# yuchencong/quantum_circuits_symmetry_breaking_based_on_tneq-qc

Hardware: NVIDIA B200
Metric: samples/sec for QCTN fwd+bwd contraction (higher is better)
Workload: dtype f32

## Files before the change

quantum_circuits_symmetry_breaking_based_on_tneq-qc_b200/csrc/tnq_ladder.cu:

```cuda
#include <cuda_runtime.h>
#include <stdint.h>
#include <stdlib.h>

#include <string>

#include "tneq_b200.h"
#include "tnq_ladder_core.cuh"

extern int tnq_internal_fail(const std::string& msg);
extern int tnq_internal_cuda_fail(cudaError_t e, const char* what);
extern void tnq_internal_count_launch();

namespace {

using namespace tnq_ladder;

constexpr int WARPS_FWD = 16;
constexpr int WARPS_TRAIN = 8;

template <int K>
__host__ __device__ constexpr int cst_floats(int n) {
    return ((n - 1) * Dims<K>::CSTEP + Dims<K>::K2 + 3) / 4 * 4;
}

template <int K, int MODE>
__global__ void __maxnreg__(MODE == 0 ? 128 : 255)
tnq_ladder_kernel(const __grid_constant__ Args a, long long B, long long ngroups, const float* __restrict__ seed,
                  float* __restrict__ values, float* __restrict__ gparts, float* __restrict__ lparts,
                  float* __restrict__ ckpt, float log_scale, float inv_count) {
    using D = Dims<K>;
    extern __shared__ __align__(16) float sm[];
    const int n = a.n;
    const int ncst = (n - 1) * D::CSTEP + D::K2;
    for (int i = threadIdx.x; i < ncst; i += blockDim.x) sm[i] = const_pool_element<K>(a, i);
    constexpr int WSZ = MODE == 0 ? D::WARP_FWD : D::WARP_TRAIN;
    const int warp = threadIdx.x >> 5, lane = threadIdx.x & 31, wpc = blockDim.x >> 5;
    float* wb = sm + cst_floats<K>(n) + warp * WSZ;
    for (int i = lane; i < WSZ; i += 32) wb[i] = 0.f;
    __syncthreads();
    const long long wg = (long long)warp * gridDim.x + blockIdx.x;
    const long long wtotal = (long long)wpc * gridDim.x;
    if (wg >= ngroups) return;
    WarpCtx<K> c;
    c.cst = sm;
    c.E = wb;
    c.U = c.E + D::E_SZ;
    c.T2 = c.U + D::U_SZ;
    c.M = c.T2 + D::T2_SZ;
    c.V = c.M + D::M_SZ;
    c.D = c.V + D::V_SZ;
    c.dT2 = c.D + D::E_SZ;
    c.args = &a;
    c.B = B;
    c.seed = seed;
    c.values = values;
    c.log_scale = log_scale;
    c.inv_count = inv_count;
    c.ckE = nullptr, c.ckT2 = nullptr, c.gpart = nullptr;
    if (MODE != 0) {
        const int ng = D::grad_floats(n);
        c.gpart = gparts + (size_t)wg * ng;
        for (int i = lane; i < ng; i += 32) c.gpart[i] = 0.f;
        c.ckE = ckpt + (size_t)wg * D::ckpt_floats(n);
        c.ckT2 = c.ckE + (size_t)(n - 2) * D::E_SZ;
        __syncwarp();
    }
    LaneState<K> st;
    st.loss = 0.f;
    st.mnext = 0.f;
    for (long long g = wg; g < ngroups; g += wtotal) ladder_group<K, MODE>(c, st, lane, g * D::SPW);
    if (MODE == 1) lparts[wg * 32 + lane] = st.loss;
}

template <int K>
__global__ void __launch_bounds__(256)
// ... 27 lines not shown
    __syncthreads();
    if (w != 0 || e >= ng) return;
    float s = 0.f;
#pragma unroll
    for (int i = 0; i < 8; ++i) s += part[i][lane];
    const int nX = (n - 1) * D::K4, nB = (n - 1) * D::K3;
    if (e < nX) {
        a.gradX[e / D::K4][e % D::K4] = s;
    } else if (e < nX + nB) {
        const int q = (e - nX) / D::K3, r = (e - nX) % D::K3;
        if (q == 0) return;
        const int cc = r / D::K2, ee = (r / K) % K, f = r % K;
        for (int d = 0; d < K; ++d) a.gradA[q][((cc * K + d) * K + ee) * K + f] = s * __ldg(a.state[q + 1] + d);
    } else if (e < nX + nB + D::K2) {
        const int ef = e - nX - nB;
        for (int cc = 0; cc < K; ++cc)
            for (int d = 0; d < K; ++d)
                a.gradA[0][(cc * K + d) * D::K2 + ef] = s * __ldg(a.state[0] + cc) * __ldg(a.state[1] + d);
    }
}

struct Geometry {
    int grid, wpc;
    long long ngroups, nwarps;
    size_t smem;
};

template <int K>
Geometry geometry(int n, long long B, int mode, int sms) {
    using D = Dims<K>;
    Geometry g;
    g.ngroups = (B + D::SPW - 1) / D::SPW;
    int wmax = mode == 0 ? WARPS_FWD : WARPS_TRAIN;
    {
        int dev = 0, smem_max = 227 * 1024;
        if (cudaGetDevice(&dev) == cudaSuccess) cudaDeviceGetAttribute(&smem_max, cudaDevAttrMaxSharedMemoryPerBlockOptin, dev);
        const long long per_warp = (long long)sizeof(float) * (mode == 0 ? D::WARP_FWD : D::WARP_TRAIN);
        const long long fit = ((long long)smem_max - (long long)sizeof(float) * cst_floats<K>(n)) / per_warp;
        if (fit < wmax) wmax = fit < 1 ? 1 : (int)fit;
    }
    long long wpc = (g.ngroups + sms - 1) / sms;
    g.wpc = (int)(wpc < 1 ? 1 : (wpc > wmax ? wmax : wpc));
    long long grid = (g.ngroups + g.wpc - 1) / g.wpc;
    g.grid = (int)(grid > sms ? sms : grid);
    g.nwarps = (long long)g.grid * g.wpc;
    if (g.nwarps > g.ngroups) g.nwarps = g.ngroups;
    g.smem = sizeof(float) * ((size_t)cst_floats<K>(n) + (size_t)g.wpc * (mode == 0 ? D::WARP_FWD : D::WARP_TRAIN));
    return g;
}

template <int K>
size_t workspace_bytes(int n, long long B, int mode, int sms) {
    using D = Dims<K>;
    if (mode == 0) return 256;
    const Geometry g = geometry<K>(n, B, mode, sms);
    const size_t nw = (size_t)g.grid * g.wpc;
    return sizeof(float) * nw * ((size_t)D::grad_floats(n) + 32 + (size_t)D::ckpt_floats(n)) + 256;
}

template <int K, int MODE>
int launch_mode(const Args& a, const Geometry& g, long long B, const float* seed, float* values, float* gparts,
                float* lparts, float* ckpt, float log_scale, cudaStream_t st) {
    cudaError_t e = cudaFuncSetAttribute(tnq_ladder_kernel<K, MODE>, cudaFuncAttributeMaxDynamicSharedMemorySize, (int)g.smem);
    if (e != cudaSuccess) return tnq_internal_cuda_fail(e, "cudaFuncSetAttribute(ladder)");
    tnq_ladder_kernel<K, MODE><<<g.grid, g.wpc * 32, g.smem, st>>>(a, B, g.ngroups, seed, values, gparts, lparts, ckpt,
                                                                    log_scale, 1.0f / (float)B);
    tnq_internal_count_launch();
    return 0;
}

template <int K>
int launch_ladder(const Args& a, long long B, int mode, const float* seed, float* values, float* loss, float log_scale,
                  void* workspace, long long ws_bytes, cudaStream_t st) {
    using D = Dims<K>;
    int dev = 0, sms = 148;
    cudaGetDevice(&dev);
    cudaDeviceGetAttribute(&sms, cudaDevAttrMultiProcessorCount, dev);
    const Geometry g = geometry<K>(a.n, B, mode, sms);
    float *gparts = nullptr, *lparts = nullptr, *ckpt = nullptr;
    if (mode != 0) {
        if ((size_t)ws_bytes < workspace_bytes<K>(a.n, B, mode, sms)) return tnq_internal_fail("tnq_mps_ladder: workspace too small");
        const size_t nw = (size_t)g.grid * g.wpc;
        gparts = reinterpret_cast<float*>(workspace);
        lparts = gparts + nw * D::grad_floats(a.n);
        ckpt = lparts + nw * 32;
    }
    int rc;
    if (mode == 0)
        rc = launch_mode<K, 0>(a, g, B, seed, values, gparts, lparts, ckpt, log_scale, st);
    else if (mode == 1)
        rc = launch_mode<K, 1>(a, g, B, seed, values, gparts, lparts, ckpt, log_scale, st);
    else
        rc = launch_mode<K, 2>(a, g, B, seed, values, gparts, lparts, ckpt, log_scale, st);
    if (rc) return rc;
    if (mode != 0) {
        const int nblk = (D::grad_floats(a.n) + 31) / 32;
        tnq_ladder_finalize_kernel<K><<<nblk + (mode == 1 ? 1 : 0), 256, 0, st>>>(a, gparts, lparts, (int)g.nwarps,
                                                                                  mode == 1 ? loss : nullptr);
        tnq_internal_count_launch();
    }
    const cudaError_t e = cudaGetLastError();
    if (e != cudaSuccess) return tnq_internal_cuda_fail(e, "tnq_mps_ladder launch");
    return 0;
}

}

extern "C" {

static bool use_second_generation(int K) {
    const char* v = getenv("TNQ_LADDER_V2");
    return K == 3 && v != nullptr && v[0] == '1';
}

int64_t tnq_mps_ladder_workspace_bytes(int K, int n, int64_t B, int mode) {
    if (use_second_generation(K)) return tnq_mps_ladder2_workspace_bytes(n, B, mode);
    int dev = 0, sms = 148;
    if (cudaGetDevice(&dev) == cudaSuccess) cudaDeviceGetAttribute(&sms, cudaDevAttrMultiProcessorCount, dev);
    if (n < 3 || n > MAXQ || B <= 0) return 256;
    return (int64_t)(K == 2 ? workspace_bytes<2>(n, B, mode, sms) : workspace_bytes<3>(n, B, mode, sms));
}

int tnq_mps_ladder(int K, int n, const float* const* cores_a, const float* const* cores_x, const float* const* states,
                   const float* const* mx, const int64_t* mx_stride, int64_t B, int mode, const float* seed,
                   float* values, float* loss, float* const* grads_a, float* const* grads_x, double log_scale,
                   void* workspace, int64_t workspace_bytes, void* stream) {
    if (use_second_generation(K))
        return tnq_mps_ladder2(n, cores_a, cores_x, states, mx, mx_stride, B, mode, seed, values, loss, grads_a, grads_x,
                               log_scale, workspace, workspace_bytes, stream);
    if (n < 3 || n > MAXQ) return tnq_internal_fail("tnq_mps_ladder: between 3 and " + std::to_string(MAXQ) + " qubits");
    if (K != 2 && K != 3) return tnq_internal_fail("tnq_mps_ladder: edge rank must be 2 or 3");
    if (!cores_a || !cores_x || !states || !mx || !mx_stride || B <= 0 || mode < 0 || mode > 2)
        return tnq_internal_fail("tnq_mps_ladder: bad arguments");
    if (mode != 0 && (!grads_a || !grads_x || !workspace)) return tnq_internal_fail("tnq_mps_ladder: gradients need grads[] and a workspace");
    if (mode == 0 && !values) return tnq_internal_fail("tnq_mps_ladder: mode 0 needs values");
    if (mode == 1 && !loss) return tnq_internal_fail("tnq_mps_ladder: mode 1 needs loss");
    if (mode == 2 && !seed) return tnq_internal_fail("tnq_mps_ladder: mode 2 needs a seed");
    Args a;
    a.n = n;
    for (int q = 0; q < MAXQ; ++q) {
        const bool hq = q < n, hc = q < n - 1;
        a.state[q] = hq ? states[q] : nullptr;
        a.mx[q] = hq ? mx[q] : nullptr;
        a.mx_stride[q] = hq ? mx_stride[q] : 0;
        a.coreA[q] = hc ? cores_a[q] : nullptr;
        a.coreX[q] = hc ? cores_x[q] : nullptr;
        a.gradA[q] = (hc && mode != 0) ? grads_a[q] : nullptr;
        a.gradX[q] = (hc && mode != 0) ? grads_x[q] : nullptr;
        if (hq && (!states[q] || !mx[q])) return tnq_internal_fail("tnq_mps_ladder: null pointer at qubit " + std::to_string(q));
        if (hc && (!cores_a[q] || !cores_x[q] || (mode != 0 && (!grads_a[q] || !grads_x[q]))))
            return tnq_internal_fail("tnq_mps_ladder: null core pointer at qubit " + std::to_string(q));
    }
    cudaStream_t st = (cudaStream_t)stream;
    if (K == 2) return launch_ladder<2>(a, B, mode, seed, values, loss, (float)log_scale, workspace, workspace_bytes, st);
    return launch_ladder<3>(a, B, mode, seed, values, loss, (float)log_scale, workspace, workspace_bytes, st);
}

}
```

quantum_circuits_symmetry_breaking_based_on_tneq-qc_b200/csrc/tnq_ladder_core.cuh:

```cuda
#pragma once

#include <math.h>
#include <stdint.h>

#ifdef __CUDACC__
#define TNQ_HOSTDEV __host__ __device__
#define TNQ_HD __device__ __forceinline__
#define TNQ_UNROLL _Pragma("unroll")
#define TNQ_NOUNROLL _Pragma("unroll 1")
#define TNQ_UNROLL3 _Pragma("unroll 3")
#else
#define TNQ_HOSTDEV
#define TNQ_HD inline
#define TNQ_UNROLL
#define TNQ_NOUNROLL
#define TNQ_UNROLL3
#endif

#include "tnq_f2.cuh"

namespace tnq_ladder {

constexpr int MAXQ = 64;

template <int K>
struct Dims {
    static constexpr int K2 = K * K, K3 = K2 * K, K4 = K2 * K2;
    static constexpr int IPS = K2;
    static constexpr int SPW = 32 / IPS;
    static constexpr int LANES = SPW * IPS;
    static constexpr int PITCH = K == 3 ? 85 : 16;
    static constexpr int SST = K == 3 ? 765 : 67;
    static constexpr int UP = 4;
    static constexpr int UQ = (K2 + 3) / 4 * 4;
    static constexpr int USZ = K3 * UP > K2 * UQ ? K3 * UP : K2 * UQ;
    static constexpr int XTP = (K2 + 3) / 4 * 4;
    static constexpr int BSP = 4;
    static constexpr int LP = LANES | 1;
    static constexpr int BTP = (K2 + 3) / 4 * 4;
    static constexpr int OFF_XN = 0, OFF_XT = (K4 + 3) / 4 * 4, OFF_BS = OFF_XT + K2 * XTP;
    static constexpr int OFF_BT = (OFF_BS + K2 * BSP + 3) / 4 * 4;
    static constexpr int CSTEP = (OFF_BT + K * BTP + 3) / 4 * 4;
    static constexpr int E_SZ = (SPW * SST + 3) / 4 * 4;
    static constexpr int U_SZ = SPW * USZ;
    static constexpr int T2_SZ = (SPW * K4 + 3) / 4 * 4;
    static constexpr int M_SZ = (SPW * K2 + 3) / 4 * 4;
    static constexpr int V_SZ = 64;
    static constexpr int WARP_FWD = E_SZ + U_SZ + T2_SZ + M_SZ + V_SZ;
    static constexpr int WARP_TRAIN = WARP_FWD + E_SZ + T2_SZ;
    static_assert(SPW * SST >= K4 * LP, "environment buffer doubles as the lane-reduction scratch");
    static_assert(USZ >= K4, "U buffer doubles as the X-gradient side buffer");
    TNQ_HOSTDEV static constexpr int ckpt_floats(int n) { return (n - 2) * (E_SZ + T2_SZ); }
    TNQ_HOSTDEV static constexpr int grad_floats(int n) { return ((n - 1) * K4 + (n - 1) * K3 + K2 + 3) / 4 * 4; }
};

struct Args {
    const float* coreA[MAXQ];
    const float* coreX[MAXQ];
    const float* state[MAXQ];
    const float* mx[MAXQ];
    long long mx_stride[MAXQ];
    float* gradA[MAXQ];
    float* gradX[MAXQ];
    int n;
};

template <int N>
struct Vec {
    static constexpr int NP = N / 2;
    F2 p[NP > 0 ? NP : 1];
    float s;
    TNQ_HD float get(int i) const { return i < 2 * NP ? ((i & 1) ? p[i >> 1].hi : p[i >> 1].lo) : s; }
    TNQ_HD void set(int i, float v) {
        if (i < 2 * NP) {
            if (i & 1) p[i >> 1].hi = v; else p[i >> 1].lo = v;
        } else {
            s = v;
        }
    }
    TNQ_HD void zero() {
        TNQ_UNROLL
        for (int i = 0; i < NP; ++i) p[i] = F2{0.f, 0.f};
        s = 0.f;
    }
};
template <int N>
TNQ_HD void axpy(Vec<N>& acc, float s, const Vec<N>& x) {
    TNQ_UNROLL
    for (int i = 0; i < Vec<N>::NP; ++i) acc.p[i] = fma2(x.p[i], s, acc.p[i]);
    if (N & 1) acc.s = fmaf(x.s, s, acc.s);
}
template <int N>
TNQ_HD float dot(const Vec<N>& a, const Vec<N>& b, float init) {
    F2 t{init, 0.f};
    TNQ_UNROLL
    for (int i = 0; i < Vec<N>::NP; ++i) t = fma2(a.p[i], b.p[i], t);
    if (N & 1) t.lo = fmaf(a.s, b.s, t.lo);
    return t.lo + t.hi;
}
template <int N>
TNQ_HD void vload(Vec<N>& v, const float* p) {
    float t[(N + 3) / 4 * 4];
#ifdef __CUDA_ARCH__
    TNQ_UNROLL
    for (int i = 0; i < (N + 3) / 4; ++i) {
        const float4 q = *reinterpret_cast<const float4*>(p + 4 * i);
        t[4 * i] = q.x, t[4 * i + 1] = q.y, t[4 * i + 2] = q.z, t[4 * i + 3] = q.w;
    }
#else
    for (int i = 0; i < (N + 3) / 4 * 4; ++i) t[i] = p[i];
#endif
    TNQ_UNROLL
    for (int i = 0; i < N; ++i) v.set(i, t[i]);
}

template <int K>
struct LaneState {
// ... 36 lines not shown
        }
    } else {
        TNQ_UNROLL
        for (int i = 0; i < N; ++i) o[i] = p[i];
    }
#else
    for (int i = 0; i < N; ++i) o[i] = p[i];
#endif
}
template <int N>
TNQ_HD void stv(float* p, const float (&o)[N]) {
#ifdef __CUDA_ARCH__
    if constexpr (N % 4 == 0) {
        TNQ_UNROLL
        for (int i = 0; i < N; i += 4) *reinterpret_cast<float4*>(p + i) = make_float4(o[i], o[i + 1], o[i + 2], o[i + 3]);
    } else if constexpr (N % 2 == 0) {
        TNQ_UNROLL
        for (int i = 0; i < N; i += 2) *reinterpret_cast<float2*>(p + i) = make_float2(o[i], o[i + 1]);
    } else {
        TNQ_UNROLL
        for (int i = 0; i < N; ++i) p[i] = o[i];
    }
#else
    for (int i = 0; i < N; ++i) p[i] = o[i];
#endif
}

TNQ_HD float ldg_f(const float* p) {
#ifdef __CUDA_ARCH__
    return __ldg(p);
#else
    return *p;
#endif
}

template <int K>
TNQ_HD float load_m(const WarpCtx<K>& c, int q, long long b, int it) {
    return b < c.B ? ldg_f(c.args->mx[q] + b * c.args->mx_stride[q] + it) : 0.f;
}

template <int K>
TNQ_HD void gather_epg(const float* e, Vec<Dims<K>::K2> (&Epg)[K][K]) {
    using D = Dims<K>;
    TNQ_UNROLL
    for (int cc = 0; cc < K; ++cc)
        TNQ_UNROLL
        for (int ee = 0; ee < K; ++ee)
            TNQ_UNROLL
            for (int l = 0; l < K; ++l)
                TNQ_UNROLL
                for (int n = 0; n < K; ++n) Epg[cc][ee].set(l * K + n, e[(cc * K + l) * D::PITCH + n * D::K3 + ee * K]);
}
template <int K>
TNQ_HD void contract_t1(const float* Bs, const Vec<Dims<K>::K2> (&Epg)[K][K], Vec<Dims<K>::K2> (&T1)[K]) {
    using D = Dims<K>;
    TNQ_UNROLL
    for (int f = 0; f < K; ++f) T1[f].zero();
    TNQ_UNROLL
    for (int cc = 0; cc < K; ++cc)
        TNQ_UNROLL
        for (int ee = 0; ee < K; ++ee) {
            float bs[D::BSP];
            ldv<D::BSP>(Bs + (cc * K + ee) * D::BSP, bs);
            TNQ_UNROLL
            for (int f = 0; f < K; ++f) axpy(T1[f], bs[f], Epg[cc][ee]);
        }
}

template <int K>
TNQ_HD void phase_a_fwd(const WarpCtx<K>& c, int lane, const float* Bs) {
    using D = Dims<K>;
    const int s = lane / D::IPS, it = lane % D::IPS, p = it / K, g = it % K;
    Vec<D::K2> Epg[K][K], T1[K];
    gather_epg<K>(c.E + s * D::SST + p * D::K2 + g, Epg);
    contract_t1<K>(Bs, Epg, T1);
    Vec<K> T2[K];
    TNQ_UNROLL
    for (int f = 0; f < K; ++f) T2[f].zero();
    TNQ_UNROLL
    for (int ln = 0; ln < D::K2; ++ln) {
        Vec<K> bs;
        vload<K>(bs, Bs + ln * D::BSP);
        TNQ_UNROLL
        for (int f = 0; f < K; ++f) axpy(T2[f], T1[f].get(ln), bs);
    }
    float* t2 = c.T2 + s * D::K4 + g * K + p;
    TNQ_UNROLL
    for (int f = 0; f < K; ++f)
        TNQ_UNROLL
        for (int o = 0; o < K; ++o) t2[(f * K + o) * D::K2] = T2[f].get(o);
}

template <int K, int LAYOUT>
TNQ_HD void phase_b(const WarpCtx<K>& c, int lane, const float* Xn) {
    using D = Dims<K>;
    const int s = lane / D::IPS, qr = lane % D::IPS, q = qr / K, r = qr % K;
    float mm[K][K];
    TNQ_UNROLL
    for (int i = 0; i < K; ++i)
        TNQ_UNROLL
        for (int k = 0; k < K; ++k) mm[i][k] = c.M[s * D::K2 + i * K + k];
    float x[K][K];
    TNQ_UNROLL
    for (int p = 0; p < K; ++p)
        TNQ_UNROLL
        for (int k = 0; k < K; ++k) x[p][k] = Xn[((p * K + q) * K + k) * K + r];
    TNQ_UNROLL
    for (int i = 0; i < K; ++i) {
        float u[D::UP];
        TNQ_UNROLL
        for (int p = 0; p < D::UP; ++p) {
            float a = 0.f;
            if (p < K) {
                TNQ_UNROLL
                for (int k = 0; k < K; ++k) a = fmaf(mm[i][k], x[p < K ? p : 0][k], a);
            }
            u[p] = a;
        }
        if (LAYOUT == 1) {
            stv<D::UP>(c.U + s * D::USZ + (i * D::K2 + qr) * D::UP, u);
        } else {
            TNQ_UNROLL
            for (int p = 0; p < K; ++p) c.U[s * D::USZ + (i * K + p) * D::UQ + qr] = u[p];
        }
    }
}

template <int K>
TNQ_HD void fill_t2_first(const WarpCtx<K>& c, int lane, const float* As0) {
    using D = Dims<K>;
    const int s = lane / D::IPS, it = lane % D::IPS, f = it / K, o = it % K;
    float* t2 = c.T2 + s * D::K4 + it * D::K2;
    TNQ_UNROLL
    for (int g = 0; g < K; ++g)
        TNQ_UNROLL
        for (int p = 0; p < K; ++p) t2[g * K + p] = As0[g * K + f] * As0[p * K + o];
}

template <int K>
TNQ_HD void phase_c_fwd(const WarpCtx<K>& c, int lane, const float* Xt) {
    using D = Dims<K>;
    const int s = lane / D::IPS, fo = lane % D::IPS;
    float t2[K][K];
    TNQ_UNROLL
    for (int g = 0; g < K; ++g)
        TNQ_UNROLL
        for (int p = 0; p < K; ++p) t2[g][p] = c.T2[s * D::K4 + fo * D::K2 + g * K + p];
    Vec<D::K2> V[D::K2];
    TNQ_UNROLL
    for (int gi = 0; gi < D::K2; ++gi) V[gi].zero();
    const float* U = c.U + s * D::USZ;
    TNQ_UNROLL
    for (int i = 0; i < K; ++i)
        TNQ_UNROLL
        for (int p = 0; p < K; ++p) {
            Vec<D::K2> u;
            vload<D::K2>(u, U + (i * K + p) * D::UQ);
            TNQ_UNROLL
            for (int g = 0; g < K; ++g) axpy(V[g * K + i], t2[g][p], u);
        }
    float* e = c.E + s * D::SST + fo * D::PITCH;
    TNQ_UNROLL
    for (int hj = 0; hj < D::K2; ++hj) {
        float xt[D::XTP];
        ldv<D::XTP>(Xt + hj * D::XTP, xt);
        Vec<D::K2> out;
        out.zero();
        TNQ_UNROLL
        for (int gi = 0; gi < D::K2; ++gi) axpy(out, xt[gi], V[gi]);
        TNQ_UNROLL
        for (int qr = 0; qr < D::K2; ++qr) e[qr * D::K2 + hj] = out.get(qr);
    }
}

template <int K>
TNQ_HD void last_p2(const WarpCtx<K>& c, int lane, const float* Xn, float (&t2)[K][K], float (&P2)[K][K][K]) {
    using D = Dims<K>;
    const int s = lane / D::IPS, fo = lane % D::IPS, o = fo % K;
    TNQ_UNROLL
    for (int g = 0; g < K; ++g)
        TNQ_UNROLL
        for (int p = 0; p < K; ++p) t2[g][p] = c.T2[s * D::K4 + fo * D::K2 + g * K + p];
    float P1[K][K][K];
    TNQ_UNROLL
    for (int j = 0; j < K; ++j)
        TNQ_UNROLL
        for (int pp = 0; pp < K; ++pp) {
            float x[K];
            TNQ_UNROLL
            for (int p0 = 0; p0 < K; ++p0) x[p0] = Xn[((p0 * K + o) * K + j) * K + pp];
            TNQ_UNROLL
            for (int g = 0; g < K; ++g) {
                float a = 0.f;
                TNQ_UNROLL
                for (int p0 = 0; p0 < K; ++p0) a = fmaf(t2[g][p0], x[p0], a);
                P1[g][j][pp] = a;
            }
        }
    TNQ_UNROLL
    for (int h = 0; h < K; ++h) {
        float m[K];
        TNQ_UNROLL
        for (int j = 0; j < K; ++j) m[j] = c.M[s * D::K2 + h * K + j];
        TNQ_UNROLL
        for (int g = 0; g < K; ++g)
            TNQ_UNROLL
            for (int pp = 0; pp < K; ++pp) {
                float a = 0.f;
                TNQ_UNROLL
                for (int j = 0; j < K; ++j) a = fmaf(m[j], P1[g][j][pp], a);
                P2[g][h][pp] = a;
            }
    }
}

template <int K>
TNQ_HD void last_fwd(const WarpCtx<K>& c, LaneState<K>& st, int lane, const float* Xn) {
    using D = Dims<K>;
    const int f = (lane % D::IPS) / K;
    float t2[K][K], P2[K][K][K];
    last_p2<K>(c, lane, Xn, t2, P2);
    TNQ_UNROLL
// ... 37 lines not shown
            TNQ_UNROLL
            for (int pp = 0; pp < K; ++pp) {
                float a = 0.f;
                TNQ_UNROLL
                for (int i = 0; i < K; ++i) a = fmaf(x[i], st.pf[i * K + pp], a);
                dP2[g][h][pp] = a;
            }
        }
    float dP1[K][K][K];
    TNQ_UNROLL
    for (int j = 0; j < K; ++j) {
        float m[K];
        TNQ_UNROLL
        for (int h = 0; h < K; ++h) m[h] = c.M[s * D::K2 + h * K + j];
        TNQ_UNROLL
        for (int g = 0; g < K; ++g)
            TNQ_UNROLL
            for (int pp = 0; pp < K; ++pp) {
                float a = 0.f;
                TNQ_UNROLL
                for (int h = 0; h < K; ++h) a = fmaf(m[h], dP2[g][h][pp], a);
                dP1[g][j][pp] = a;
            }
    }
    float dt2[K][K];
    TNQ_UNROLL
    for (int g = 0; g < K; ++g)
        TNQ_UNROLL
        for (int p0 = 0; p0 < K; ++p0) dt2[g][p0] = 0.f;
    TNQ_UNROLL
    for (int p0 = 0; p0 < K; ++p0)
        TNQ_UNROLL
        for (int j = 0; j < K; ++j)
            TNQ_UNROLL
            for (int pp = 0; pp < K; ++pp) {
                const float x = Xn[((p0 * K + o) * K + j) * K + pp];
                float cx = 0.f;
                TNQ_UNROLL
                for (int g = 0; g < K; ++g) {
                    dt2[g][p0] = fmaf(dP1[g][j][pp], x, dt2[g][p0]);
                    cx = fmaf(t2[g][p0], dP1[g][j][pp], cx);
                }
                TNQ_UNROLL
                for (int O = 0; O < K; ++O)
                    st.accX[p0 * K + j].set(O * K + pp, st.accX[p0 * K + j].get(O * K + pp) + ((O == o) ? cx : 0.f));
            }
    TNQ_UNROLL
    for (int g = 0; g < K; ++g)
        TNQ_UNROLL
        for (int p0 = 0; p0 < K; ++p0) c.dT2[s * D::K4 + fo * D::K2 + g * K + p0] = dt2[g][p0];
}

template <int K>
TNQ_HD void phase_c_bwd(const WarpCtx<K>& c, LaneState<K>& st, int lane, const float* Xt) {
    using D = Dims<K>;
    const int s = lane / D::IPS, fo = lane % D::IPS;
    Vec<K> t2T[K], dt2[K];
    TNQ_UNROLL
    for (int g = 0; g < K; ++g) {
        dt2[g].zero();
        TNQ_UNROLL
        for (int p = 0; p < K; ++p) t2T[p].set(g, c.T2[s * D::K4 + fo * D::K2 + g * K + p]);
    }
    TNQ_UNROLL
    for (int v = 0; v < D::K2; ++v) st.accX[v].zero();
    const float* U = c.U + s * D::USZ;
    float* d = c.D + s * D::SST + fo * D::PITCH;
    TNQ_NOUNROLL
    for (int qr = 0; qr < D::K2; ++qr) {
        Vec<K> u[K];
        TNQ_UNROLL
        for (int i = 0; i < K; ++i) vload<K>(u[i], U + (i * D::K2 + qr) * D::UP);
        Vec<D::K2> de;
        TNQ_UNROLL
        for (int hj = 0; hj < D::K2; ++hj) de.set(hj, d[qr * D::K2 + hj]);
        TNQ_UNROLL
        for (int i = 0; i < K; ++i) {
            Vec<K> v;
            v.zero();
            TNQ_UNROLL
            for (int p = 0; p < K; ++p) axpy(v, u[i].get(p), t2T[p]);
            TNQ_UNROLL
            for (int g = 0; g < K; ++g) axpy(st.accX[g * K + i], v.get(g), de);
        }
        Vec<D::K2> z;
        z.zero();
        TNQ_UNROLL
        for (int hj = 0; hj < D::K2; ++hj) {
            Vec<D::K2> xt;
            vload<D::K2>(xt, Xt + hj * D::XTP);
            axpy(z, de.get(hj), xt);
        }
        TNQ_UNROLL
        for (int g = 0; g < K; ++g)
            TNQ_UNROLL
            for (int i = 0; i < K; ++i) {
                axpy(dt2[g], z.get(g * K + i), u[i]);
                d[qr * D::K2 + g * K + i] = z.get(g * K + i);
            }
    }
    TNQ_UNROLL
    for (int g = 0; g < K; ++g)
        TNQ_UNROLL
        for (int p = 0; p < K; ++p) c.dT2[s * D::K4 + fo * D::K2 + g * K + p] = dt2[g].get(p);
}

template <int K>
TNQ_HD void phase_du(const WarpCtx<K>& c, int lane) {
    using D = Dims<K>;
    const int s = lane / D::IPS, qr = lane % D::IPS, q = qr / K, r = qr % K;
    Vec<K> du[K];
    TNQ_UNROLL
    for (int i = 0; i < K; ++i) du[i].zero();
    const float* z = c.D + s * D::SST + qr * D::K2;
    const float* t2 = c.T2 + s * D::K4;
    TNQ_UNROLL
    for (int fo = 0; fo < D::K2; ++fo)
        TNQ_UNROLL
        for (int g = 0; g < K; ++g) {
            Vec<K> tt;
            TNQ_UNROLL
            for (int p = 0; p < K; ++p) tt.set(p, t2[fo * D::K2 + g * K + p]);
            TNQ_UNROLL
            for (int i = 0; i < K; ++i) axpy(du[i], z[fo * D::PITCH + g * K + i], tt);
        }
    float* xr = c.U + s * D::USZ;
    TNQ_UNROLL
    for (int k = 0; k < K; ++k) {
        Vec<K> w;
        w.zero();
        TNQ_UNROLL
        for (int i = 0; i < K; ++i) axpy(w, c.M[s * D::K2 + i * K + k], du[i]);
        TNQ_UNROLL
        for (int p = 0; p < K; ++p) xr[((p * K + q) * K + k) * K + r] = w.get(p);
    }
}

template <int K>
TNQ_HD void phase_a_bwd(const WarpCtx<K>& c, LaneState<K>& st, int lane, const float* Bs, const float* BsT) {
    using D = Dims<K>;
    const int s = lane / D::IPS, it = lane % D::IPS, p = it / K, g = it % K;
    Vec<D::K2> Epg[K][K], T1[K], X2[K];
    gather_epg<K>(c.E + s * D::SST + p * D::K2 + g, Epg);
    Vec<K> dt[K];
    TNQ_UNROLL
    for (int f = 0; f < K; ++f)
        TNQ_UNROLL
        for (int o = 0; o < K; ++o) dt[f].set(o, c.dT2[s * D::K4 + (f * K + o) * D::K2 + g * K + p]);
    contract_t1<K>(Bs, Epg, T1);
    TNQ_UNROLL
    for (int ln = 0; ln < D::K2; ++ln) {
        st.accB[ln].zero();
        TNQ_UNROLL
        for (int f = 0; f < K; ++f) axpy(st.accB[ln], T1[f].get(ln), dt[f]);
    }
    TNQ_UNROLL
    for (int f = 0; f < K; ++f) X2[f].zero();
    TNQ_UNROLL
    for (int o = 0; o < K; ++o) {
        Vec<D::K2> bt;
        vload<D::K2>(bt, BsT + o * D::BTP);
        TNQ_UNROLL
        for (int f = 0; f < K; ++f) axpy(X2[f], dt[f].get(o), bt);
    }
    float* d = c.D + s * D::SST + p * D::K2 + g;
    TNQ_UNROLL
    for (int cc = 0; cc < K; ++cc)
        TNQ_UNROLL
        for (int ee = 0; ee < K; ++ee) {
            float bs[D::BSP];
            ldv<D::BSP>(Bs + (cc * K + ee) * D::BSP, bs);
            Vec<D::K2> de;
            de.zero();
            TNQ_UNROLL
            for (int f = 0; f < K; ++f) {
                axpy(de, bs[f], X2[f]);
                st.accB[cc * K + ee].set(f, dot(Epg[cc][ee], X2[f], st.accB[cc * K + ee].get(f)));
            }
            TNQ_UNROLL
            for (int l = 0; l < K; ++l)
                TNQ_UNROLL
                for (int n = 0; n < K; ++n) d[(cc * K + l) * D::PITCH + n * D::K3 + ee * K] = de.get(l * K + n);
        }
}

template <int K>
TNQ_HD void first_a_bwd(const WarpCtx<K>& c, LaneState<K>& st, int lane, const float* As0) {
    using D = Dims<K>;
    const int s = lane / D::IPS, fo = lane % D::IPS, f = fo / K, o = fo % K;
    TNQ_UNROLL
    for (int v = 0; v < K; ++v) st.accB[v].zero();
    float dt[K][K];
    TNQ_UNROLL
    for (int g = 0; g < K; ++g)
        TNQ_UNROLL
        for (int p = 0; p < K; ++p) dt[g][p] = c.dT2[s * D::K4 + fo * D::K2 + g * K + p];
    TNQ_UNROLL
    for (int g = 0; g < K; ++g) {
        float cl = 0.f;
        TNQ_UNROLL
        for (int p = 0; p < K; ++p) cl = fmaf(dt[g][p], As0[p * K + o], cl);
        TNQ_UNROLL
        for (int F = 0; F < K; ++F) st.accB[g].set(F, st.accB[g].get(F) + ((F == f) ? cl : 0.f));
    }
    TNQ_UNROLL
    for (int p = 0; p < K; ++p) {
        float cr = 0.f;
        TNQ_UNROLL
        for (int g = 0; g < K; ++g) cr = fmaf(dt[g][p], As0[g * K + f], cr);
        TNQ_UNROLL
        for (int O = 0; O < K; ++O) st.accB[p].set(O, st.accB[p].get(O) + ((O == o) ? cr : 0.f));
    }
}

TNQ_HD void gadd(float* p, float v) {
#ifdef __CUDA_ARCH__
    atomicAdd(p, v);
#else
    *p += v;
#endif
}

template <int K>
TNQ_HD void flush_put_x(float* scr, int lane, const Vec<Dims<K>::K2> (&acc)[Dims<K>::K2]) {
    using D = Dims<K>;
    TNQ_UNROLL
    for (int g = 0; g < K; ++g)
        TNQ_UNROLL
        for (int h = 0; h < K; ++h)
// ... 45 lines not shown
#ifdef __CUDA_ARCH__
    const uint32_t d = (uint32_t)__cvta_generic_to_shared(dst);
    TNQ_UNROLL
    for (int i = 0; i < (NFLOATS / 4 + 31) / 32; ++i) {
        const int j = lane + 32 * i;
        if (j < NFLOATS / 4)
            asm volatile("cp.async.cg.shared.global [%0], [%1], 16;" ::"r"(d + 16u * j), "l"(src + 4 * j) : "memory");
    }
#else
    for (int i = lane; i < NFLOATS; i += 32) dst[i] = src[i];
#endif
}
TNQ_HD void ckpt_commit() {
#ifdef __CUDA_ARCH__
    asm volatile("cp.async.commit_group;" ::: "memory");
#endif
}
template <int PENDING>
TNQ_HD void ckpt_wait() {
#ifdef __CUDA_ARCH__
    asm volatile("cp.async.wait_group %0;" ::"n"(PENDING) : "memory");
#endif
}

}

#ifdef __CUDACC__
#define TNQ_PHASE(...) \
    { __VA_ARGS__ }    \
    __syncwarp();
#define TNQ_LANES_PARAM LaneState<K>&st, const int lane
#else
#define TNQ_PHASE(...)                         \
    for (int lane = 0; lane < 32; ++lane) {    \
        LaneState<K>& st = lanes[lane];        \
        (void)st;                              \
        __VA_ARGS__                            \
    }
#define TNQ_LANES_PARAM LaneState<K>* lanes
#endif

namespace tnq_ladder {

template <int K, int MODE>
TNQ_HD void ladder_group(const WarpCtx<K>& c, TNQ_LANES_PARAM, long long b0) {
    using D = Dims<K>;
    const int n = c.args->n;
    const float* As0 = c.cst + (n - 1) * D::CSTEP;
    constexpr bool CK = MODE != 0;
#define TNQ_ACTIVE (lane < D::LANES)
#define TNQ_S (lane / D::IPS)
#define TNQ_IT (lane % D::IPS)
#define TNQ_XN(q) (c.cst + (q) * D::CSTEP + D::OFF_XN)
#define TNQ_XT(q) (c.cst + (q) * D::CSTEP + D::OFF_XT)
#define TNQ_BS(q) (c.cst + (q) * D::CSTEP + D::OFF_BS)
#define TNQ_BT(q) (c.cst + (q) * D::CSTEP + D::OFF_BT)
#define TNQ_GX(q) (c.gpart + (q) * D::K4)
#define TNQ_GB(q) (c.gpart + (n - 1) * D::K4 + (q) * D::K3)
#define TNQ_GA0 (c.gpart + (n - 1) * D::K4 + (n - 1) * D::K3)

    TNQ_PHASE(if (TNQ_ACTIVE) {
        c.M[lane] = load_m<K>(c, 0, b0 + TNQ_S, TNQ_IT);
        st.mnext = load_m<K>(c, 1, b0 + TNQ_S, TNQ_IT);
        fill_t2_first<K>(c, lane, As0);
    })
    TNQ_PHASE(if (TNQ_ACTIVE) phase_b<K, 2>(c, lane, TNQ_XN(0));)
    TNQ_PHASE(if (TNQ_ACTIVE) phase_c_fwd<K>(c, lane, TNQ_XT(0));)
    for (int q = 1; q <= n - 2; ++q) {
        TNQ_PHASE(
            if (CK && q < n - 2) ckpt_store<D::E_SZ>(c.ckE + (size_t)(q - 1) * D::E_SZ, c.E, lane);
            if (TNQ_ACTIVE) {
                c.M[lane] = st.mnext;
                st.mnext = load_m<K>(c, q + 1, b0 + TNQ_S, TNQ_IT);
                phase_a_fwd<K>(c, lane, TNQ_BS(q));
            })
        if (q < n - 2) {
            TNQ_PHASE(
                if (CK) ckpt_store<D::T2_SZ>(c.ckT2 + (size_t)(q - 1) * D::T2_SZ, c.T2, lane);
                if (TNQ_ACTIVE) phase_b<K, 2>(c, lane, TNQ_XN(q));)
            TNQ_PHASE(if (TNQ_ACTIVE) phase_c_fwd<K>(c, lane, TNQ_XT(q));)
        }
    }
    TNQ_PHASE(if (TNQ_ACTIVE) last_fwd<K>(c, st, lane, TNQ_XN(n - 2));)
    TNQ_PHASE(if (TNQ_ACTIVE) c.M[lane] = st.mnext;)
    TNQ_PHASE(if (TNQ_ACTIVE) {
        float v = 0.f;
        const float* m = c.M + TNQ_S * D::K2;
        TNQ_UNROLL
        for (int i = 0; i < D::K2; ++i) v = fmaf(st.pf[i], m[i], v);
        c.V[lane] = v;
    })
    TNQ_PHASE(if (TNQ_ACTIVE && TNQ_IT == 0) {
        float val = 0.f;
        TNQ_UNROLL
        for (int i = 0; i < D::IPS; ++i) val += c.V[lane + i];
        const long long b = b0 + TNQ_S;
        const bool valid = b < c.B;
        if (MODE != 2 && valid && c.values != nullptr) c.values[b] = val;
        float dv = 0.f;
        if (MODE == 1) {
            const float cl = val > 1e-10f ? val : 1e-10f;
            if (valid) {
                st.loss -= (logf(cl) + c.log_scale) * c.inv_count;
                dv = val >= 1e-10f ? -c.inv_count / cl : 0.f;
            }
        } else if (MODE == 2) {
            dv = valid ? ldg_f(c.seed + b) : 0.f;
        }
        c.V[32 + TNQ_S] = dv;
    })
    if (MODE == 0) return;

    TNQ_PHASE(if (TNQ_ACTIVE) {
        const float dv = c.V[32 + TNQ_S];
        const float* m = c.M + TNQ_S * D::K2;
        TNQ_UNROLL
        for (int i = 0; i < D::K2; ++i) st.pf[i] = dv * m[i];
        st.mnext = load_m<K>(c, n - 2, b0 + TNQ_S, TNQ_IT);
    })
    TNQ_PHASE(if (TNQ_ACTIVE) {
        c.M[lane] = st.mnext;
        if (n >= 3) st.mnext = load_m<K>(c, n - 3, b0 + TNQ_S, TNQ_IT);
    })
    TNQ_PHASE(if (TNQ_ACTIVE) {
        last_bwd<K>(c, st, lane, TNQ_XN(n - 2));
        flush_put_x<K>(c.D, lane, st.accX);
    })
    TNQ_PHASE(
        flush_sum<K, D::K4, false>(c.D, nullptr, lane, TNQ_GX(n - 2));
        if (n - 3 >= 1) ckpt_load_async<D::T2_SZ>(c.T2, c.ckT2 + (size_t)(n - 4) * D::T2_SZ, lane);
        ckpt_commit();)
    for (int q = n - 2; q >= 1; --q) {
        if (q < n - 2) {
            TNQ_PHASE(
                ckpt_load_async<D::E_SZ>(c.E, c.ckE + (size_t)(q - 1) * D::E_SZ, lane);
                ckpt_commit();
                if (TNQ_ACTIVE) {
                    c.M[lane] = st.mnext;
                    st.mnext = load_m<K>(c, q - 1, b0 + TNQ_S, TNQ_IT);
                })
            TNQ_PHASE(
                if (TNQ_ACTIVE) phase_b<K, 1>(c, lane, TNQ_XN(q));
                ckpt_wait<1>();)
            TNQ_PHASE(if (TNQ_ACTIVE) phase_c_bwd<K>(c, st, lane, TNQ_XT(q));)
            TNQ_PHASE(if (TNQ_ACTIVE) phase_du<K>(c, lane);)
            TNQ_PHASE(
                if (TNQ_ACTIVE) flush_put_x<K>(c.D, lane, st.accX);
                if (q - 1 >= 1) ckpt_load_async<D::T2_SZ>(c.T2, c.ckT2 + (size_t)(q - 2) * D::T2_SZ, lane);
                ckpt_commit();)
            TNQ_PHASE(
                flush_sum<K, D::K4, true>(c.D, c.U, lane, TNQ_GX(q));
                ckpt_wait<1>();)
        }
        TNQ_PHASE(if (TNQ_ACTIVE) phase_a_bwd<K>(c, st, lane, TNQ_BS(q), TNQ_BT(q));)
        TNQ_PHASE(if (TNQ_ACTIVE) flush_put_b<K, D::K2>(c.E, lane, st.accB);)
        TNQ_PHASE(flush_sum<K, D::K3, false>(c.E, nullptr, lane, TNQ_GB(q));)
    }
    TNQ_PHASE(ckpt_wait<0>();)
    TNQ_PHASE(if (TNQ_ACTIVE) {
        c.M[lane] = st.mnext;
        fill_t2_first<K>(c, lane, As0);
    })
    TNQ_PHASE(if (TNQ_ACTIVE) phase_b<K, 1>(c, lane, TNQ_XN(0));)
    TNQ_PHASE(if (TNQ_ACTIVE) phase_c_bwd<K>(c, st, lane, TNQ_XT(0));)
    TNQ_PHASE(if (TNQ_ACTIVE) phase_du<K>(c, lane);)
    TNQ_PHASE(if (TNQ_ACTIVE) flush_put_x<K>(c.D, lane, st.accX);)
    TNQ_PHASE(flush_sum<K, D::K4, true>(c.D, c.U, lane, TNQ_GX(0));)
    TNQ_PHASE(if (TNQ_ACTIVE) {
        first_a_bwd<K>(c, st, lane, As0);
        flush_put_b<K, K>(c.E, lane, st.accB);
    })
    TNQ_PHASE(flush_sum<K, D::K2, false>(c.E, nullptr, lane, TNQ_GA0);)
#undef TNQ_ACTIVE
#undef TNQ_S
#undef TNQ_IT
#undef TNQ_XN
#undef TNQ_XT
#undef TNQ_BS
#undef TNQ_BT
#undef TNQ_GX
#undef TNQ_GB
#undef TNQ_GA0
}

template <int K>
TNQ_HD float const_pool_element(const Args& a, int idx) {
    using D = Dims<K>;
    const int n = a.n;
    if (idx >= (n - 1) * D::CSTEP) {
        const int ef = idx - (n - 1) * D::CSTEP;
        float v = 0.f;
        for (int cc = 0; cc < K; ++cc)
            for (int d = 0; d < K; ++d) v = fmaf(a.coreA[0][(cc * K + d) * D::K2 + ef], a.state[0][cc] * a.state[1][d], v);
        return v;
    }
    const int q = idx / D::CSTEP, r = idx % D::CSTEP;
    if (r < D::OFF_XT) return a.coreX[q][r];
    if (r < D::OFF_BS) {
        const int hj = (r - D::OFF_XT) / D::XTP, gi = (r - D::OFF_XT) % D::XTP;
        if (gi >= D::K2) return 0.f;
        const int h = hj / K, j = hj % K, g = gi / K, i = gi % K;
        return a.coreX[q][((g * K + h) * K + i) * K + j];
    }
    if (q == 0) return 0.f;
    int ce, f;
    if (r < D::OFF_BT) {
        const int t = r - D::OFF_BS;
        if (t >= D::K2 * D::BSP) return 0.f;
        ce = t / D::BSP, f = t % D::BSP;
    } else {
        const int t = r - D::OFF_BT;
        if (t >= K * D::BTP) return 0.f;
        f = t / D::BTP, ce = t % D::BTP;
    }
    if (f >= K || ce >= D::K2) return 0.f;
    const int cc = ce / K, e = ce % K;
    float v = 0.f;
    for (int d = 0; d < K; ++d) v = fmaf(a.coreA[q][((cc * K + d) * K + e) * K + f], a.state[q + 1][d], v);
    return v;
}

template <int K>
TNQ_HD float grad_element(const Args& a, const float* gparts, int nwarps, int layer, int q, int v) {
    using D = Dims<K>;
    const int n = a.n, stride = D::grad_floats(n);
    int off;
    float w = 1.f;
    if (layer == 1) {
        off = q * D::K4 + v;
    } else {
        const int f = v % K, e = (v / K) % K, d = (v / D::K2) % K, cc = v / D::K3;
        if (q == 0) {
            off = (n - 1) * D::K4 + (n - 1) * D::K3 + e * K + f;
            w = a.state[0][cc] * a.state[1][d];
        } else {
            off = (n - 1) * D::K4 + q * D::K3 + (cc * K + e) * K + f;
            w = a.state[q + 1][d];
        }
    }
    float t = 0.f;
    for (int i = 0; i < nwarps; ++i) t += gparts[(size_t)i * stride + off];
    return t * w;
}

}
```

Baseline: 13.82 million.

## Serve warp-uniform ladder constants (Xt, Bs, Bt) from __constant__ memory image

Adds a prep kernel that builds the Xt/Bs/BsT constant coefficients into a workspace image, copies it into a __constant__ array with cudaMemcpyToSymbolAsync, and makes the contraction phases read those coefficients through the constant cache instead of shared memory via a CStep accessor. The intent is to replace shared-memory vector loads of warp-uniform operands with constant-bank operands that FMAs can use directly, cutting shared-memory traffic and registers. It adds a prep kernel and memcpy per call, a global event to serialize use of the single constant image across streams, and requires a workspace in forward mode too. Constant reads are only fast when all lanes hit the same address, and the added launches cost more when batches are small.

```diff
diff --git a/quantum_circuits_symmetry_breaking_based_on_tneq-qc_b200/csrc/tnq_ladder.cu b/quantum_circuits_symmetry_breaking_based_on_tneq-qc_b200/csrc/tnq_ladder.cu
--- a/quantum_circuits_symmetry_breaking_based_on_tneq-qc_b200/csrc/tnq_ladder.cu
+++ b/quantum_circuits_symmetry_breaking_based_on_tneq-qc_b200/csrc/tnq_ladder.cu
@@ -2,9 +2,11 @@
 #include <stdint.h>
 #include <stdlib.h>
 
+#include <mutex>
 #include <string>
 
 #include "tneq_b200.h"
+#define TNQ_LADDER_CIMG
 #include "tnq_ladder_core.cuh"
 
 extern int tnq_internal_fail(const std::string& msg);
@@ -21,6 +23,28 @@
 template <int K>
 __host__ __device__ constexpr int cst_floats(int n) {
     return ((n - 1) * Dims<K>::CSTEP + Dims<K>::K2 + 3) / 4 * 4;
+}
+
+template <int K>
+__host__ __device__ constexpr int img_floats(int n) {
+    return (n - 1) * Dims<K>::CIMG;
+}
+constexpr size_t IMG_BYTES = (sizeof(float) * CIMG_FLOATS + 255) / 256 * 256;
+
+template <int K>
+__global__ void __launch_bounds__(256) tnq_ladder_prep_kernel(const __grid_constant__ Args a, float* __restrict__ image) {
+    const int i = blockIdx.x * blockDim.x + threadIdx.x;
+    if (i < img_floats<K>(a.n)) image[i] = cimg_element<K>(a, i);
+}
+
+struct ImageOrder {
+    std::mutex mu;
+    cudaEvent_t ev[64] = {};
+    bool recorded[64] = {};
+};
+ImageOrder& image_order() {
+    static ImageOrder o;
+    return o;
 }
 
 template <int K, int MODE>
@@ -154,10 +178,10 @@
 template <int K>
 size_t workspace_bytes(int n, long long B, int mode, int sms) {
     using D = Dims<K>;
-    if (mode == 0) return 256;
+    if (mode == 0) return IMG_BYTES + 256;
     const Geometry g = geometry<K>(n, B, mode, sms);
     const size_t nw = (size_t)g.grid * g.wpc;
-    return sizeof(float) * nw * ((size_t)D::grad_floats(n) + 32 + (size_t)D::ckpt_floats(n)) + 256;
+    return IMG_BYTES + sizeof(float) * nw * ((size_t)D::grad_floats(n) + 32 + (size_t)D::ckpt_floats(n)) + 256;
 }
 
 template <int K, int MODE>
@@ -179,14 +203,37 @@
     cudaGetDevice(&dev);
     cudaDeviceGetAttribute(&sms, cudaDevAttrMultiProcessorCount, dev);
     const Geometry g = geometry<K>(a.n, B, mode, sms);
+    if ((size_t)ws_bytes < workspace_bytes<K>(a.n, B, mode, sms)) return tnq_internal_fail("tnq_mps_ladder: workspace too small");
+    float* image = reinterpret_cast<float*>(workspace);
     float *gparts = nullptr, *lparts = nullptr, *ckpt = nullptr;
     if (mode != 0) {
-        if ((size_t)ws_bytes < workspace_bytes<K>(a.n, B, mode, sms)) return tnq_internal_fail("tnq_mps_ladder: workspace too small");
         const size_t nw = (size_t)g.grid * g.wpc;
-        gparts = reinterpret_cast<float*>(workspace);
+        gparts = reinterpret_cast<float*>(static_cast<char*>(workspace) + IMG_BYTES);
         lparts = gparts + nw * D::grad_floats(a.n);
         ckpt = lparts + nw * 32;
     }
+    if (dev < 0 || dev >= 64) return tnq_internal_fail("tnq_mps_ladder: device index out of range");
+    ImageOrder& o = image_order();
+    std::lock_guard<std::mutex> lock(o.mu);
+    cudaError_t e;
+    if (o.ev[dev] == nullptr) {
+        e = cudaEventCreateWithFlags(&o.ev[dev], cudaEventDisableTiming);
+        if (e != cudaSuccess) return tnq_internal_cuda_fail(e, "cudaEventCreate(ladder constant image)");
+    }
+    cudaStreamCaptureStatus cs = cudaStreamCaptureStatusNone;
+    e = cudaStreamIsCapturing(st, &cs);
+    if (e != cudaSuccess) return tnq_internal_cuda_fail(e, "cudaStreamIsCapturing(ladder)");
+    const bool capturing = cs == cudaStreamCaptureStatusActive;
+    if (o.recorded[dev]) {
+        e = cudaStreamWaitEvent(st, o.ev[dev], capturing ? cudaEventWaitExternal : 0);
+        if (e != cudaSuccess) return tnq_internal_cuda_fail(e, "cudaStreamWaitEvent(ladder constant image)");
+    }
+    const int ni = img_floats<K>(a.n);
+    tnq_ladder_prep_kernel<K><<<(ni + 255) / 256, 256, 0, st>>>(a, image);
+    tnq_internal_count_launch();
+    e = cudaMemcpyToSymbolAsync(ladder_cimg, image, sizeof(float) * ni, 0, cudaMemcpyDeviceToDevice, st);
+    if (e != cudaSuccess) return tnq_internal_cuda_fail(e, "cudaMemcpyToSymbolAsync(ladder constant image)");
+    tnq_internal_count_launch();
     int rc;
     if (mode == 0)
         rc = launch_mode<K, 0>(a, g, B, seed, values, gparts, lparts, ckpt, log_scale, st);
@@ -195,13 +242,16 @@
     else
         rc = launch_mode<K, 2>(a, g, B, seed, values, gparts, lparts, ckpt, log_scale, st);
     if (rc) return rc;
+    e = capturing ? cudaEventRecordWithFlags(o.ev[dev], st, cudaEventRecordExternal) : cudaEventRecord(o.ev[dev], st);
+    if (e != cudaSuccess) return tnq_internal_cuda_fail(e, "cudaEventRecord(ladder constant image)");
+    o.recorded[dev] = true;
     if (mode != 0) {
         const int nblk = (D::grad_floats(a.n) + 31) / 32;
         tnq_ladder_finalize_kernel<K><<<nblk + (mode == 1 ? 1 : 0), 256, 0, st>>>(a, gparts, lparts, (int)g.nwarps,
                                                                                   mode == 1 ? loss : nullptr);
         tnq_internal_count_launch();
     }
-    const cudaError_t e = cudaGetLastError();
+    e = cudaGetLastError();
     if (e != cudaSuccess) return tnq_internal_cuda_fail(e, "tnq_mps_ladder launch");
     return 0;
 }
@@ -234,7 +284,8 @@
     if (K != 2 && K != 3) return tnq_internal_fail("tnq_mps_ladder: edge rank must be 2 or 3");
     if (!cores_a || !cores_x || !states || !mx || !mx_stride || B <= 0 || mode < 0 || mode > 2)
         return tnq_internal_fail("tnq_mps_ladder: bad arguments");
-    if (mode != 0 && (!grads_a || !grads_x || !workspace)) return tnq_internal_fail("tnq_mps_ladder: gradients need grads[] and a workspace");
+    if (!workspace) return tnq_internal_fail("tnq_mps_ladder: needs a workspace (the constant image lives there)");
+    if (mode != 0 && (!grads_a || !grads_x)) return tnq_internal_fail("tnq_mps_ladder: gradients need grads[]");
     if (mode == 0 && !values) return tnq_internal_fail("tnq_mps_ladder: mode 0 needs values");
     if (mode == 1 && !loss) return tnq_internal_fail("tnq_mps_ladder: mode 1 needs loss");
     if (mode == 2 && !seed) return tnq_internal_fail("tnq_mps_ladder: mode 2 needs a seed");
diff --git a/quantum_circuits_symmetry_breaking_based_on_tneq-qc_b200/csrc/tnq_ladder_core.cuh b/quantum_circuits_symmetry_breaking_based_on_tneq-qc_b200/csrc/tnq_ladder_core.cuh
--- a/quantum_circuits_symmetry_breaking_based_on_tneq-qc_b200/csrc/tnq_ladder_core.cuh
+++ b/quantum_circuits_symmetry_breaking_based_on_tneq-qc_b200/csrc/tnq_ladder_core.cuh
@@ -41,6 +41,8 @@
     static constexpr int OFF_XN = 0, OFF_XT = (K4 + 3) / 4 * 4, OFF_BS = OFF_XT + K2 * XTP;
     static constexpr int OFF_BT = (OFF_BS + K2 * BSP + 3) / 4 * 4;
     static constexpr int CSTEP = (OFF_BT + K * BTP + 3) / 4 * 4;
+    static constexpr int CIMG = CSTEP - OFF_XT;
+    static constexpr int IMG_XT = 0, IMG_BS = OFF_BS - OFF_XT, IMG_BT = OFF_BT - OFF_XT;
     static constexpr int E_SZ = (SPW * SST + 3) / 4 * 4;
     static constexpr int U_SZ = SPW * USZ;
     static constexpr int T2_SZ = (SPW * K4 + 3) / 4 * 4;
@@ -63,6 +65,26 @@
     float* gradA[MAXQ];
     float* gradX[MAXQ];
     int n;
+};
+
+constexpr int CIMG_FLOATS = (MAXQ - 1) * Dims<3>::CIMG;
+static_assert(CIMG_FLOATS * sizeof(float) <= 65536, "the constant image of MAXQ qubits fits one 64 KB bank");
+static_assert((MAXQ - 1) * Dims<2>::CIMG <= CIMG_FLOATS, "K = 2 uses the same image");
+#if defined(__CUDACC__) && defined(TNQ_LADDER_CIMG)
+#define TNQ_CIMG_DEVICE 1
+__constant__ float ladder_cimg[CIMG_FLOATS];
+#else
+#define TNQ_CIMG_DEVICE 0
+#endif
+
+struct CStep {
+#if TNQ_CIMG_DEVICE
+    int base;
+    TNQ_HD float operator[](int i) const { return ladder_cimg[base + i]; }
+#else
+    const float* p;
+    TNQ_HD float operator[](int i) const { return p[i]; }
+#endif
 };
 
 template <int N>
@@ -205,35 +227,33 @@
                 for (int n = 0; n < K; ++n) Epg[cc][ee].set(l * K + n, e[(cc * K + l) * D::PITCH + n * D::K3 + ee * K]);
 }
 template <int K>
-TNQ_HD void contract_t1(const float* Bs, const Vec<Dims<K>::K2> (&Epg)[K][K], Vec<Dims<K>::K2> (&T1)[K]) {
+TNQ_HD void contract_t1(const CStep& X, const Vec<Dims<K>::K2> (&Epg)[K][K], Vec<Dims<K>::K2> (&T1)[K]) {
     using D = Dims<K>;
     TNQ_UNROLL
     for (int f = 0; f < K; ++f) T1[f].zero();
     TNQ_UNROLL
     for (int cc = 0; cc < K; ++cc)
         TNQ_UNROLL
-        for (int ee = 0; ee < K; ++ee) {
-            float bs[D::BSP];
-            ldv<D::BSP>(Bs + (cc * K + ee) * D::BSP, bs);
-            TNQ_UNROLL
-            for (int f = 0; f < K; ++f) axpy(T1[f], bs[f], Epg[cc][ee]);
-        }
-}
-
-template <int K>
-TNQ_HD void phase_a_fwd(const WarpCtx<K>& c, int lane, const float* Bs) {
+        for (int ee = 0; ee < K; ++ee)
+            TNQ_UNROLL
+            for (int f = 0; f < K; ++f) axpy(T1[f], X[D::IMG_BS + (cc * K + ee) * D::BSP + f], Epg[cc][ee]);
+}
+
+template <int K>
+TNQ_HD void phase_a_fwd(const WarpCtx<K>& c, int lane, const CStep& X) {
     using D = Dims<K>;
     const int s = lane / D::IPS, it = lane % D::IPS, p = it / K, g = it % K;
     Vec<D::K2> Epg[K][K], T1[K];
     gather_epg<K>(c.E + s * D::SST + p * D::K2 + g, Epg);
-    contract_t1<K>(Bs, Epg, T1);
+    contract_t1<K>(X, Epg, T1);
     Vec<K> T2[K];
     TNQ_UNROLL
     for (int f = 0; f < K; ++f) T2[f].zero();
     TNQ_UNROLL
     for (int ln = 0; ln < D::K2; ++ln) {
         Vec<K> bs;
-        vload<K>(bs, Bs + ln * D::BSP);
+        TNQ_UNROLL
+        for (int o = 0; o < K; ++o) bs.set(o, X[D::IMG_BS + ln * D::BSP + o]);
         TNQ_UNROLL
         for (int f = 0; f < K; ++f) axpy(T2[f], T1[f].get(ln), bs);
     }
@@ -291,7 +311,7 @@
 }
 
 template <int K>
-TNQ_HD void phase_c_fwd(const WarpCtx<K>& c, int lane, const float* Xt) {
+TNQ_HD void phase_c_fwd(const WarpCtx<K>& c, int lane, const CStep& X) {
     using D = Dims<K>;
     const int s = lane / D::IPS, fo = lane % D::IPS;
     float t2[K][K];
@@ -315,12 +335,10 @@
     float* e = c.E + s * D::SST + fo * D::PITCH;
     TNQ_UNROLL
     for (int hj = 0; hj < D::K2; ++hj) {
-        float xt[D::XTP];
-        ldv<D::XTP>(Xt + hj * D::XTP, xt);
         Vec<D::K2> out;
         out.zero();
         TNQ_UNROLL
-        for (int gi = 0; gi < D::K2; ++gi) axpy(out, xt[gi], V[gi]);
+        for (int gi = 0; gi < D::K2; ++gi) axpy(out, X[D::IMG_XT + hj * D::XTP + gi], V[gi]);
         TNQ_UNROLL
         for (int qr = 0; qr < D::K2; ++qr) e[qr * D::K2 + hj] = out.get(qr);
     }
@@ -464,7 +482,7 @@
 }
 
 template <int K>
-TNQ_HD void phase_c_bwd(const WarpCtx<K>& c, LaneState<K>& st, int lane, const float* Xt) {
+TNQ_HD void phase_c_bwd(const WarpCtx<K>& c, LaneState<K>& st, int lane, const CStep& X) {
     using D = Dims<K>;
     const int s = lane / D::IPS, fo = lane % D::IPS;
     Vec<K> t2T[K], dt2[K];
@@ -500,7 +518,8 @@
         TNQ_UNROLL
         for (int hj = 0; hj < D::K2; ++hj) {
             Vec<D::K2> xt;
-            vload<D::K2>(xt, Xt + hj * D::XTP);
+            TNQ_UNROLL
+            for (int gi = 0; gi < D::K2; ++gi) xt.set(gi, X[D::IMG_XT + hj * D::XTP + gi]);
             axpy(z, de.get(hj), xt);
         }
         TNQ_UNROLL
@@ -549,7 +568,7 @@
 }
 
 template <int K>
-TNQ_HD void phase_a_bwd(const WarpCtx<K>& c, LaneState<K>& st, int lane, const float* Bs, const float* BsT) {
+TNQ_HD void phase_a_bwd(const WarpCtx<K>& c, LaneState<K>& st, int lane, const CStep& X) {
     using D = Dims<K>;
     const int s = lane / D::IPS, it = lane % D::IPS, p = it / K, g = it % K;
     Vec<D::K2> Epg[K][K], T1[K], X2[K];
@@ -559,7 +578,7 @@
     for (int f = 0; f < K; ++f)
         TNQ_UNROLL
         for (int o = 0; o < K; ++o) dt[f].set(o, c.dT2[s * D::K4 + (f * K + o) * D::K2 + g * K + p]);
-    contract_t1<K>(Bs, Epg, T1);
+    contract_t1<K>(X, Epg, T1);
     TNQ_UNROLL
     for (int ln = 0; ln < D::K2; ++ln) {
         st.accB[ln].zero();
@@ -571,7 +590,8 @@
     TNQ_UNROLL
     for (int o = 0; o < K; ++o) {
         Vec<D::K2> bt;
-        vload<D::K2>(bt, BsT + o * D::BTP);
+        TNQ_UNROLL
+        for (int ln = 0; ln < D::K2; ++ln) bt.set(ln, X[D::IMG_BT + o * D::BTP + ln]);
         TNQ_UNROLL
         for (int f = 0; f < K; ++f) axpy(X2[f], dt[f].get(o), bt);
     }
@@ -580,13 +600,11 @@
     for (int cc = 0; cc < K; ++cc)
         TNQ_UNROLL
         for (int ee = 0; ee < K; ++ee) {
-            float bs[D::BSP];
-            ldv<D::BSP>(Bs + (cc * K + ee) * D::BSP, bs);
             Vec<D::K2> de;
             de.zero();
             TNQ_UNROLL
             for (int f = 0; f < K; ++f) {
-                axpy(de, bs[f], X2[f]);
+                axpy(de, X[D::IMG_BS + (cc * K + ee) * D::BSP + f], X2[f]);
                 st.accB[cc * K + ee].set(f, dot(Epg[cc][ee], X2[f], st.accB[cc * K + ee].get(f)));
             }
             TNQ_UNROLL
@@ -738,9 +756,11 @@
 #define TNQ_S (lane / D::IPS)
 #define TNQ_IT (lane % D::IPS)
 #define TNQ_XN(q) (c.cst + (q) * D::CSTEP + D::OFF_XN)
-#define TNQ_XT(q) (c.cst + (q) * D::CSTEP + D::OFF_XT)
-#define TNQ_BS(q) (c.cst + (q) * D::CSTEP + D::OFF_BS)
-#define TNQ_BT(q) (c.cst + (q) * D::CSTEP + D::OFF_BT)
+#if TNQ_CIMG_DEVICE
+#define TNQ_IMG(q) (CStep{(q) * D::CIMG})
+#else
+#define TNQ_IMG(q) (CStep{c.cst + (q) * D::CSTEP + D::OFF_XT})
+#endif
 #define TNQ_GX(q) (c.gpart + (q) * D::K4)
 #define TNQ_GB(q) (c.gpart + (n - 1) * D::K4 + (q) * D::K3)
 #define TNQ_GA0 (c.gpart + (n - 1) * D::K4 + (n - 1) * D::K3)
@@ -751,20 +771,20 @@
         fill_t2_first<K>(c, lane, As0);
     })
     TNQ_PHASE(if (TNQ_ACTIVE) phase_b<K, 2>(c, lane, TNQ_XN(0));)
-    TNQ_PHASE(if (TNQ_ACTIVE) phase_c_fwd<K>(c, lane, TNQ_XT(0));)
+    TNQ_PHASE(if (TNQ_ACTIVE) phase_c_fwd<K>(c, lane, TNQ_IMG(0));)
     for (int q = 1; q <= n - 2; ++q) {
         TNQ_PHASE(
             if (CK && q < n - 2) ckpt_store<D::E_SZ>(c.ckE + (size_t)(q - 1) * D::E_SZ, c.E, lane);
             if (TNQ_ACTIVE) {
                 c.M[lane] = st.mnext;
                 st.mnext = load_m<K>(c, q + 1, b0 + TNQ_S, TNQ_IT);
-                phase_a_fwd<K>(c, lane, TNQ_BS(q));
+                phase_a_fwd<K>(c, lane, TNQ_IMG(q));
             })
         if (q < n - 2) {
             TNQ_PHASE(
                 if (CK) ckpt_store<D::T2_SZ>(c.ckT2 + (size_t)(q - 1) * D::T2_SZ, c.T2, lane);
                 if (TNQ_ACTIVE) phase_b<K, 2>(c, lane, TNQ_XN(q));)
-            TNQ_PHASE(if (TNQ_ACTIVE) phase_c_fwd<K>(c, lane, TNQ_XT(q));)
+            TNQ_PHASE(if (TNQ_ACTIVE) phase_c_fwd<K>(c, lane, TNQ_IMG(q));)
         }
     }
     TNQ_PHASE(if (TNQ_ACTIVE) last_fwd<K>(c, st, lane, TNQ_XN(n - 2));)
@@ -828,7 +848,7 @@
             TNQ_PHASE(
                 if (TNQ_ACTIVE) phase_b<K, 1>(c, lane, TNQ_XN(q));
                 ckpt_wait<1>();)
-            TNQ_PHASE(if (TNQ_ACTIVE) phase_c_bwd<K>(c, st, lane, TNQ_XT(q));)
+            TNQ_PHASE(if (TNQ_ACTIVE) phase_c_bwd<K>(c, st, lane, TNQ_IMG(q));)
             TNQ_PHASE(if (TNQ_ACTIVE) phase_du<K>(c, lane);)
             TNQ_PHASE(
                 if (TNQ_ACTIVE) flush_put_x<K>(c.D, lane, st.accX);
@@ -838,7 +858,7 @@
                 flush_sum<K, D::K4, true>(c.D, c.U, lane, TNQ_GX(q));
                 ckpt_wait<1>();)
         }
-        TNQ_PHASE(if (TNQ_ACTIVE) phase_a_bwd<K>(c, st, lane, TNQ_BS(q), TNQ_BT(q));)
+        TNQ_PHASE(if (TNQ_ACTIVE) phase_a_bwd<K>(c, st, lane, TNQ_IMG(q));)
         TNQ_PHASE(if (TNQ_ACTIVE) flush_put_b<K, D::K2>(c.E, lane, st.accB);)
         TNQ_PHASE(flush_sum<K, D::K3, false>(c.E, nullptr, lane, TNQ_GB(q));)
     }
@@ -848,7 +868,7 @@
         fill_t2_first<K>(c, lane, As0);
     })
     TNQ_PHASE(if (TNQ_ACTIVE) phase_b<K, 1>(c, lane, TNQ_XN(0));)
-    TNQ_PHASE(if (TNQ_ACTIVE) phase_c_bwd<K>(c, st, lane, TNQ_XT(0));)
+    TNQ_PHASE(if (TNQ_ACTIVE) phase_c_bwd<K>(c, st, lane, TNQ_IMG(0));)
     TNQ_PHASE(if (TNQ_ACTIVE) phase_du<K>(c, lane);)
     TNQ_PHASE(if (TNQ_ACTIVE) flush_put_x<K>(c.D, lane, st.accX);)
     TNQ_PHASE(flush_sum<K, D::K4, true>(c.D, c.U, lane, TNQ_GX(0));)
@@ -861,9 +881,7 @@
 #undef TNQ_S
 #undef TNQ_IT
 #undef TNQ_XN
-#undef TNQ_XT
-#undef TNQ_BS
-#undef TNQ_BT
+#undef TNQ_IMG
 #undef TNQ_GX
 #undef TNQ_GB
 #undef TNQ_GA0
@@ -904,6 +922,12 @@
     float v = 0.f;
     for (int d = 0; d < K; ++d) v = fmaf(a.coreA[q][((cc * K + d) * K + e) * K + f], a.state[q + 1][d], v);
     return v;
+}
+
+template <int K>
+TNQ_HD float cimg_element(const Args& a, int i) {
+    using D = Dims<K>;
+    return const_pool_element<K>(a, (i / D::CIMG) * D::CSTEP + D::OFF_XT + i % D::CIMG);
 }
 
 template <int K>
```

Result: faster. 14.92 million, median of 6 (+8.0%).
